# hiimmuc/SpeakerVerification

Hardware: AMD Instinct MI355X
Metric: embeddings/sec (2 s @16 kHz) (higher is better)
Workload: dtype bf16

## Files before the change

### speakerverification_amd/csrc/api.hip

```cpp
#include <algorithm>
#include <cstdlib>
#include <cstring>

#include "handle.h"

using namespace svhip;

namespace svhip {
RaggedCheckFn ecapa_ragged_check, rawnet2_ragged_check, rawnet3_ragged_check, conformer_ragged_check, titanet_ragged_check, resnetse_ragged_check;
RaggedEmbedFn ecapa_embed_ragged, rawnet2_embed_ragged, rawnet3_embed_ragged, conformer_embed_ragged, titanet_embed_ragged, resnetse_embed_ragged;
}

namespace {

thread_local std::string g_create_error;

enum DevOptParse { OPT_NO_ENV, OPT_SET, OPT_IS1, OPT_NUM };
struct DevOptRow { const char* name; int svhip_handle::DevOpts::*field; const char* env; DevOptParse parse; int dflt; };
#define SV_OPT(name, env, parse, dflt) {#name, &svhip_handle::DevOpts::name, env, parse, dflt}
const DevOptRow kDevOpts[] = {
    SV_OPT(layer_labels, "SVHIP_LAYER_LABELS", OPT_SET, 0),
    SV_OPT(x3_keep_f32, "SVHIP_X3_KEEP_F32", OPT_SET, 0),
    SV_OPT(r2_big, "SVHIP_R2_BIG", OPT_IS1, 0),
    SV_OPT(asp_v1, "SVHIP_ASP_V1", OPT_IS1, 0),
// ... 5 lines not shown
    SV_OPT(asnorm_norefit, nullptr, OPT_NO_ENV, 0),
    SV_OPT(rn_sinc_full, "SVHIP_RN_SINC_FULL", OPT_IS1, 0),
    SV_OPT(fbank32, "SVHIP_FBANK32", OPT_IS1, 0),
    SV_OPT(fbank_unfused, "SVHIP_FBANK_UNFUSED", OPT_IS1, 0),
    SV_OPT(pw3_cus, "SVHIP_PW3_CUS", OPT_NUM, -1),
    SV_OPT(pw3_tail_off, "SVHIP_PW3_TAIL_OFF", OPT_IS1, 0),
    SV_OPT(cv_off, "SVHIP_CV_OFF", OPT_IS1, 0),
    SV_OPT(n128_off, "SVHIP_N128_OFF", OPT_IS1, 0),
    SV_OPT(rn_pool_off, "SVHIP_RN_POOL_OFF", OPT_IS1, 0),
    SV_OPT(rn_step_off, "SVHIP_RN_STEP_OFF", OPT_IS1, 0),
    SV_OPT(rn_sinc_f32, "SVHIP_RN_SINC_F32", OPT_IS1, 0),
    SV_OPT(rn_tail_big, "SVHIP_RN_TAIL_BIG", OPT_IS1, 0),
    SV_OPT(r2_slices, "SVHIP_R2_SLICES", OPT_NUM, -1),
    SV_OPT(rn_conv_unfused, "SVHIP_RN_CONV_UNFUSED", OPT_IS1, 0),
    SV_OPT(rn_keep, "SVHIP_RN_KEEP", OPT_IS1, 0),
};
#undef SV_OPT

int none_check(const svhip_config& c, const char*& err) {
    if (c.compute == SVHIP_F16) { err = "SVHIP_F16 is RawNet2's 16-bit mode (ECAPA's is SVHIP_BF16)"; return SVHIP_ERR_UNSUPPORTED; }
    return SVHIP_OK;
}
int fbank_then_features(svhip_handle* h, const float* d_wav, int B);

const ModelOps kModels[] = {
    {SVHIP_MODEL_ECAPA,        ecapa_check,     ecapa_spec,     ecapa_finalize,     ecapa_alloc,     ecapa_embed_wave,    ecapa_forward,     ecapa_stage,     2,
     nullptr, ecapa_ragged_check, ecapa_embed_ragged},
    {SVHIP_MODEL_RAWNET2,      rawnet2_check,   rawnet2_spec,   rawnet2_finalize,   rawnet2_alloc,   rawnet2_forward,     nullptr,           rawnet2_stage,   4},
    {SVHIP_MODEL_RAWNET2_CONV, rawnet2_check,   rawnet2_spec,   rawnet2_finalize,   rawnet2_alloc,   rawnet2_forward,     nullptr,           rawnet2_stage,   4,
     nullptr, rawnet2_ragged_check, rawnet2_embed_ragged},
// ... 661 lines not shown
```

### speakerverification_amd/csrc/api_ecapa.hip

```cpp
#include <algorithm>

#include "handle.h"

namespace svhip {

namespace {

struct EcapaState : ModelState {
    ConvLayer blocks0, mfa, asp_tdnn, asp_conv;
    ConvLayer tdnn1[3], tdnn2[3], res2[3][7];
    LinearLayer se1[3], se2[3], asp_ctx, fc;
    float* se2T[3] = {};
    void *se1_bf[3] = {}, *se2T_bf[3] = {};
    float *aspbn_scale = nullptr, *aspbn_shift = nullptr;

    bool xin_ready = false;
    bool x0_is_s32 = false;
    bool cat_f32_stale = false;
    bool h2_is_s32 = false;
    bool h1_split = false;
    void* cat_s32 = nullptr;
    void* h2_s32 = nullptr;
    void* u_s32[2] = {};
    void* X0 = nullptr;
    void *H1 = nullptr, *H2 = nullptr, *H3 = nullptr;
    void* CAT = nullptr;
    void* MFA = nullptr;
    void* ATT = nullptr;
    float* LOGITS = nullptr;
    float *d_mean = nullptr, *d_s1 = nullptr, *d_s2 = nullptr, *d_gstats = nullptr, *d_ctx = nullptr;
    float *d_pool_raw = nullptr, *d_pool_bn = nullptr;

    RagTables rag;
    float* rag_stats = nullptr;
};
// ... 208 lines not shown
            GemmParams q = conv_params(h, L, us[(j - 1) & 1], C8, h2s + (size_t)j * C8 * 4, C, M, T);
            q.W = L.Ws32; q.Wrows = L.N; q.x3 = 2; q.act1 = ACT_RELU;
            if (j < 7) { q.R = static_cast<const float*>(H1) + (size_t)(j + 1) * C8; q.ldr = C; q.Y2 = us[j & 1]; q.lda2 = C8; }
            return q;
        };
        GemmParams p2 = conv_params(h, s.tdnn2[i], H2, C, H3, C, M, T);
        p2.act1 = ACT_GELU;
        p2.colsum = cs_base; p2.colsum_stride = h->colsum_region;
        const bool r2_small = h->x3 && h2s && us[0] && us[1] && s.res2[i][0].Ws32 && !h->opt.r2_big && r2_step_supported(step_params(1)) &&
                              conv_plan(h, s.tdnn2[i], p2, h2s, C).x3;
        const bool r2_plan = r2_small || (h->x3 && h2s && us[0] && us[1] && s.res2[i][0].Ws32 && gemm_pw3r2_supported(step_params(1)));
        GemmParams p1 = tdnn1_params(i, (s32_only && (i > 0 || x0_s32)) ? nullptr : xin, ldin);
        if (r2_plan) {
            p1.side_a = h2s; p1.side_lda = C; p1.side_b = us[0]; p1.side_ldb = C8; p1.side_c = C8;
        }
        GemmPlan g1;
        if ((rc = conv_gemm(h, s.tdnn1[i], p1, xin32, ldin32, &g1))) return rc;
        if (i == 2) { s.h2_is_s32 = r2_plan; s.h1_split = r2_plan && g1.side; }
        if (r2_plan) {
            if (!g1.side) {
                if ((rc = run(h, "split_s32", 0, [&]() { return launch_split_s32(static_cast<const float*>(H1), C, h2s, M, C8, st, C); }))) return rc;
                if ((rc = run(h, "split_s32", 0, [&]() { return launch_split_s32(static_cast<const float*>(H1) + C8, C, us[0], M, C8, st, C8); }))) return rc;
            }
            for (int j = 1; j < 8; ++j) {
                const GemmParams q = step_params(j);
                if (r2_small) {
                    if ((rc = run(h, "r2_step", (double)M * s.res2[i][j - 1].flops_per_row, [&]() { return launch_r2_step(q, st); }))) return rc;
                } else if ((rc = run(h, "gemm_pw3r2", (double)M * s.res2[i][j - 1].flops_per_row, [&]() { return launch_gemm_pw3r2(q, st); }))) return rc;
            }
            p2.A = nullptr;
        } else if (bf && res2net_chain_supported(C, T, s.res2[i][0].dil, s.res2[i][0].Kp)) {
            Res2Params rp;
            rp.H1 = H1; rp.H2 = H2; rp.ld = C; rp.T = T; rp.dil = s.res2[i][0].dil; rp.Kp = s.res2[i][0].Kp;
            rp.slices = h->opt.r2_slices >= 0 ? std::max(1, h->opt.r2_slices) : res2net_chain_slices(B, C, T, rp.dil, h->num_cu);
            double fl = 0;
            for (int j = 0; j < 7; ++j) {
                rp.W[j] = s.res2[i][j].W; rp.bias[j] = s.res2[i][j].bias;
                rp.scale[j] = s.res2[i][j].scale; rp.shift[j] = s.res2[i][j].shift;
                fl += (double)M * s.res2[i][j].flops_per_row;
            }
            if ((rc = run(h, rp.slices > 1 ? "res2net_slices" : "res2net_chain", fl, [&]() { return launch_res2net_chain(rp, B, C, st); }))) return rc;
        } else {
            if ((rc = run(h, "copy_cols", 0, [&]() { return launch_copy_cols(H1, C, H2, C, bf, M, C8, st); }))) return rc;
            for (int j = 1; j < 8; ++j) {
                GemmParams p = conv_params(h, s.res2[i][j - 1], off(H1, (size_t)j * C8, e), C, off(H2, (size_t)j * C8, e), C, M, T);
                p.act1 = ACT_RELU;
                p.A2 = j >= 2 ? off(H2, (size_t)(j - 1) * C8, e) : nullptr; p.lda2 = C;
                if ((rc = conv_gemm(h, s.res2[i][j - 1], p))) return rc;
// ... 59 lines not shown
        GemmParams p = conv_params(h, s.asp_conv, ATT, 128, LOGITS, C3, M, T);
        p.out_f32 = 1;
        if ((rc = conv_gemm(h, s.asp_conv, p))) return rc;
        if ((rc = run(h, "asp_pool", 0, [&]() {
                 return launch_asp_pool(LOGITS, MFA, bf, C3, B, T, C3, s.aspbn_scale, s.aspbn_shift, d_pool_raw, d_pool_bn, 1e-12f, 0.0f, st);
             }))) return rc;
    }
    if ((rc = run(h, "fc", 2.0 * B * s.fc.N * s.fc.K, [&]() {
             return launch_rowvec_linear(d_pool_bn, 2 * C3, s.fc.W, s.fc.bias, d_emb, c.embed_dim, B, c.embed_dim, 2 * C3, ACT_NONE, st, h->d_lin_part + (size_t)b0 * h->lin_part_per_utt);
         }))) return rc;
    return SVHIP_OK;
}

int ecapa_forward(svhip_handle* h, const float* d_feat, int B) {
    S(h).cat_f32_stale = false;
    const bool two = h->lanes == 2 && B >= 64 && !h->x3;
    return forward_lanes(h, ecapa_forward_part, d_feat, B, two ? 2 : 1, (B / 2 + 3) & ~3);
}

int ecapa_embed_wave(svhip_handle* h, const float* d_wav, int B) {
    auto& s = S(h);
    const int L = h->cfg.samples, T = h->T;
    const bool fused = h->bf16 && !h->in_w && h->d_logmel && !h->opt.fbank_unfused && !h->opt.fbank32 && fbank_fused_supported(h->fb, L);
    int rc;
    if (fused) {
        if ((rc = run(h, "fbank_fused", 0, [&]() {
                 return launch_fbank_fused(h->fb, d_wav, B, L, T, h->cfg.log_input, h->d_logmel, h->d_fpart, h->X_in, h->stream);
             }))) return rc;
    } else if ((rc = run(h, "fbank", 0, [&]() { return launch_fbank(h->fb, d_wav, B, L, T, h->d_feat, h->stream); }))) return rc;
    s.xin_ready = fused;
// ... 77 lines not shown
         }))) return rc;
    return run(h, "rag_fc", 2.0 * n * s.fc.N * s.fc.K, [&]() {
        return launch_rag_linear(s.d_pool_bn, 2 * C3, s.fc.W, s.fc.bias, h->d_emb, c.embed_dim, n, c.embed_dim, 2 * C3, ACT_NONE, st);
    });
}

int ecapa_embed_ragged(svhip_handle* h, const float* in, bool in_host, bool is_wave, const int64_t* in_off, const int32_t* lengths, int n) {
    auto& s = S(h);
    const size_t B = h->cfg.max_batch, utt_cap[RAG_LEVELS] = {B * (size_t)h->T};
    RagPack pk;
    int rc;
    if (!s.rag_stats && (rc = dev_alloc(h, &s.rag_stats, B * h->cfg.n_mels * 2))) return rc;
    if ((rc = rag_pack(h, s.rag, kEcapaRag, utt_cap, in, in_host, is_wave, in_off, lengths, n, pk)) || (rc = ecapa_forward_ragged(h, pk))) return rc;
    set_rag_rows(h, pk);
    s.x0_is_s32 = s.cat_f32_stale = s.h2_is_s32 = s.h1_split = false;
    return SVHIP_OK;
}

int ecapa_stage(svhip_handle* h, const std::string& n, bool fill, StageView& v) {
    auto& s = S(h);
    const int C = h->cfg.channels, C3 = 3 * C, B = h->lastB;
    const int64_t M = (int64_t)B * h->T;
    if (n == "blocks.0") {
        v.src = s.X0; v.cols = v.ld = C;
        if (s.x0_is_s32 && fill) {
            SV_HIP(h, launch_unsplit_s32(s.X0, C, static_cast<float*>(h->s32_buf), C, M, C, h->stream));
            v.src = h->s32_buf;
        }
    } else if (n == "blocks.1" || n == "blocks.2" || n == "blocks.3") {
        const int i = n.back() - '1';
        v.src = off(s.CAT, (size_t)i * C, h->esz); v.cols = C; v.ld = C3;
        if (s.cat_f32_stale && fill) {
            SV_HIP(h, launch_unsplit_s32(s.cat_s32, C3, static_cast<float*>(s.CAT), C3, M, C3, h->stream));
            s.cat_f32_stale = false;
        }
    }
    else if (n == "blocks.3.tdnn1") {
        if (s.h1_split)
            SV_FAIL(h, SVHIP_ERR_STATE, "stage blocks.3.tdnn1: the last forward wrote its first two chunks only in the split layout of the "
                                        "Res2Net step kernels, which the chain then overwrote");
        v.src = s.H1; v.cols = v.ld = C;
    } else if (n == "blocks.3.res2net") {
        v.src = s.H2; v.cols = v.ld = C;
        if (s.h2_is_s32 && fill) {
            SV_HIP(h, launch_unsplit_s32(s.h2_s32, C, static_cast<float*>(h->s32_buf), C, M, C, h->stream));
            v.src = h->s32_buf;
        }
    }
    else if (n == "blocks.3.tdnn2") { v.src = s.H3; v.cols = v.ld = C; }
    else if (n == "blocks.3.se_gate") { v.src = s.d_s2; v.rows = B; v.cols = v.ld = C; v.f32 = true; }
    else if (n == "asp_gstats") { v.src = s.d_gstats; v.rows = B; v.cols = v.ld = 2 * C3; v.f32 = true; }
    else if (n == "asp_att") { v.src = s.ATT; v.cols = v.ld = 128; }
    else if (n == "mfa") { v.src = s.MFA; v.cols = v.ld = C3; }
    else if (n == "asp") { v.src = s.d_pool_raw; v.rows = B; v.cols = v.ld = 2 * C3; v.f32 = true; }
    else if (n == "asp_bn") { v.src = s.d_pool_bn; v.rows = B; v.cols = v.ld = 2 * C3; v.f32 = true; }
    else return unknown_stage(h, n);
// ... 5 lines not shown
```

### speakerverification_amd/csrc/api_gemm.hip

```cpp
#include "handle.h"

namespace svhip {

static const void* zero_page_for(const svhip_handle* h, const void* A) {
    const char* a = static_cast<const char*>(A);
    for (const TailedBuf& b : h->tailed)
        if (a >= b.base && a < b.base + b.bytes) return b.base + b.bytes;
    return h->d_zero;
}

GemmParams conv_params(const svhip_handle* h, const ConvLayer& L, const void* A, int lda, void* Y, int ldy, int M, int T) {
    GemmParams p;
    p.A = A; p.lda = lda; p.Y = Y; p.ldy = ldy;
    p.W = L.W; p.Wrows = L.Np; p.bias = L.bias; p.scale = L.scale; p.shift = L.shift;
    p.M = M; p.N = L.N; p.K = L.K; p.Kp = L.Kp; p.T = T; p.taps = L.taps; p.dil = L.dil; p.cin = L.cin;
    p.num_cu = h->num_cu; p.pw3_cus = h->opt.pw3_cus; p.tail_split = h->opt.pw3_tail_off ? 0 : 1;
    p.zeros = h->d_zeros; p.ones = h->d_ones; p.f16 = h->f16 ? 1 : 0;
    p.cv_off = h->opt.cv_off; p.n128_off = h->opt.n128_off;
    return p;
}

GemmPlan conv_plan(const svhip_handle* h, const ConvLayer& L, GemmParams p, const void* A_s32, int lda_s32) {
    GemmPlan g;
    p.zero_page = zero_page_for(h, p.A);
    const int M = p.M;
    const bool bf = h->bf16;
    g.flops = (double)M * (L.flops_per_row + 2.0 * L.N * p.K3);
    if (h->x3 && L.Ws32 && h->s32_buf && !p.A2 && !p.bias_utt && !p.out_f32 && !p.R) {
        GemmParams q = p;
        q.A = A_s32 ? A_s32 : h->s32_buf; q.lda = A_s32 ? lda_s32 : L.K; q.W = L.Ws32; q.x3 = 2;
        if (!gemm_pw3x3_supported(q)) q.side_a = q.side_b = nullptr, q.side_c = 0;
        if (!gemm_pw3x3_supported(q) && q.colsum) q.colsum = nullptr;
        if (gemm_pw3x3_supported(q)) {
            g.q = q; g.x3 = true; g.side = q.side_c != 0; g.colsum_groups = q.colsum ? 2 : 0;
            snprintf(g.label, sizeof(g.label), "gemm_pw3x3");
            return g;
        }
    }
    if (h->x3) {
        p.x3 = 1;
        if (gemm_pw_supported(p, false) && L.Wsplit) p.W = L.Wsplit;
    }
    if (p.colsum) {
        if (gemm_pw2_supported(p, bf) && p.taps == 1) g.colsum_groups = gemm_colsum_groups(p, bf);
        else p.colsum = nullptr;
    }
    g.q = p;
    const GemmRoute route = g.route = gemm_route(p, bf);
    const char* klabel = route == ROUTE_PW3 ? "gemm_pw3" : route == ROUTE_PW3CV ? "gemm_pw3cv16" : route == ROUTE_N128 ? "gemm_n128" : route == ROUTE_PW2 ? (L.taps > 1 ? "gemm_pw2_conv" : "gemm_pw2")
                         : L.taps > 1 ? (p.A2 ? "gemm_conv_add" : "gemm_conv") : (route == ROUTE_GENERIC ? "gemm_generic" : "gemm_pw");
    if (!h->opt.layer_labels) snprintf(g.label, sizeof(g.label), "%s", klabel);
    else if (!p.K3) snprintf(g.label, sizeof(g.label), "%s M%d N%d K%d", klabel, M, L.N, L.K);
    else snprintf(g.label, sizeof(g.label), "%s M%d N%d K%d+%d", klabel, M, L.N, L.K, p.K3);
    return g;
}

int conv_gemm(svhip_handle* h, const ConvLayer& L, const GemmParams& p, const void* A_s32, int lda_s32, GemmPlan* plan) {
    const GemmPlan g = conv_plan(h, L, p, A_s32, lda_s32);
    if (plan) *plan = g;
    hipStream_t st = h->cur;
    if (g.x3) {
        int rc = A_s32 ? SVHIP_OK
                       : run(h, "split_s32", 0, [&]() { return launch_split_s32(reinterpret_cast<const float*>(p.A), p.lda, h->s32_buf, p.M, L.K, st); });
        return rc ? rc : run(h, g.label, g.flops, [&]() { return launch_gemm_pw3x3(g.q, st); });
    }
    if (!p.A)
// ... 7 lines not shown
```

### speakerverification_amd/csrc/gemm_pw3.hip

```cpp
#include <stdlib.h>

#include <type_traits>

#include "common.h"
#include "kernels.h"
#include "gemm_epi.h"

namespace svhip {

namespace {

typedef __attribute__((address_space(3))) void lds_void;
typedef __attribute__((address_space(1))) const void gbl_void;

constexpr int HT = 16384;
constexpr int RING = 8 * HT;
constexpr int CST = 3072;
constexpr int PW3_LDS = RING + 2 * CST;
constexpr int PGROUP_M = 8;

#ifdef SVHIP_GEMM_DEBUG
constexpr bool DBG3 = true;
#else
constexpr bool DBG3 = false;
#endif
#ifdef PW3_ABL
constexpr int ABL = PW3_ABL;
#else
constexpr int ABL = 0;
#endif

template <int EPI, int CS, bool X3, bool R2 = false, bool CV = false, typename H = bf16_t>
__global__ __launch_bounds__(512, 2) void gemm_pw3_kernel(GemmParams p) {
    static_assert(!R2 || (X3 && CS == 0), "the Res2Net step form exists for the X3 kernel only");
    static_assert(!CV || !R2, "the conv-gather form (CV) is the pointwise kernel with gathered X rows");
    typedef typename std::conditional<X3, x3_t, H>::type MH;
    constexpr bool GATHER = R2 || CV;
    extern __shared__ __attribute__((aligned(16))) char smem[];
    constexpr int NST = (X3 ? 32 : 16) + 8 * CS;
    constexpr int ESZ = X3 ? 4 : 2;

    const int ntm = (p.M + 255) / 256, ntn = (p.N + 255) / 256;
    const int ntiles = ntm * ntn;
    const int G = gridDim.x;
    int perm = blockIdx.x;
    {
        const int q = G >> 3, r = G & 7, xcd = perm & 7;
        perm = (xcd < r ? xcd * (q + 1) : r * (q + 1) + (xcd - r) * q) + (perm >> 3);
    }
    constexpr bool SPLIT_OK = !R2 && !(X3 && CV);
    const int qfull = (ntiles / G) * G;
    const int rtail = ntiles - qfull;
    const bool split = SPLIT_OK && p.tail_split && rtail > 0 && 2 * rtail <= G;
    const int nitems = split ? qfull + 2 * rtail : ntiles;
    auto item_tile = [&](int w, int& hsel) {
// ... 62 lines not shown
            uint32_t o = ty < 2 ? xo[ty][jj] : wo[ty - 2][jj];
            if (gather) {
                const int t = (int)((xt[jj] >> (ty * 16)) & 0xffffu);
                if (CV && !X3) {
                    const int tt = t + shift;
                    const int d = zero_pad ? shift : reflect_idx(tt, p.T) - t;
                    const uint32_t oo = (uint32_t)((int)o + d * p.lda * ESZ);
                    o = (zero_pad && (unsigned)tt >= (unsigned)p.T) ? zoff : oo;
                } else {
                    const int d = reflect_idx(t + shift, p.T) - t;
                    o = (uint32_t)((int)o + d * p.lda * ESZ);
                }
            }
            asm volatile("" : "+v"(o));
            const char* s = ub + o;
            if (!(ABL & 2)) __builtin_amdgcn_global_load_lds((gbl_void*)s, (lds_void*)(base + dsto[jj]), 16, 0, 0);
        }
    };
    auto issue_consts = [&](int n0, int par) {
        if (wave < 3) {
            const float* s = (wave == 0 ? p.bias : wave == 1 ? p.scale : p.shift) + min(n0 + lane_now() * 4, p.N - 4);
            __builtin_amdgcn_global_load_lds((gbl_void*)s, (lds_void*)(smem + RING + par * CST + wave * 1024), 16, 0, 0);
        }
    };
    auto issue_prologue = [&]() {
        issue(2, 0); issue(0, 0); issue(3, 0); issue(1, 0);
        issue(2, 1); issue(0, 1); issue(3, 1);
    };
    auto wait_left = [&](int left) {
        if (left >= 5) asm volatile("s_waitcnt vmcnt(10)" ::: "memory");
        else if (left == 4) asm volatile("s_waitcnt vmcnt(8)" ::: "memory");
// ... 296 lines not shown
                    const int m = m0 + wm * 128 + i * 16 + r16e;
                    const bool in = m < p.M && !(ABL & 8);
                    if (side_chunk < 2) {
                        uint32_t hd[2], ld[2];
#pragma unroll
                        for (int d = 0; d < 2; ++d) x3_split2(v[2 * d], v[2 * d + 1], hd[d], ld[d]);
                        const auto s0 = __builtin_amdgcn_permlane16_swap(hd[0], ld[0], false, false);
                        const auto s1 = __builtin_amdgcn_permlane16_swap(hd[1], ld[1], false, false);
                        if (in) *reinterpret_cast<u32x4*>(sbase + (int64_t)m * sld + boff) = u32x4{s0[0], s1[0], s0[1], s1[1]};
                    } else if (in) {
                        *reinterpret_cast<f32x4*>(yl + (int64_t)i * 16 * p.ldy) = v;
                    }
                }
            }
        } else {
            char* Yb = reinterpret_cast<char*>(p.Y);
#pragma unroll
            for (int jp = 0; jp < 2; ++jp) {
                if (half && jp == 1) break;
                f32x4 sc[2], sh[2];
#pragma unroll
                for (int jj = 0; jj < 2; ++jj) {
                    const int nl = wn * 64 + (2 * jp + jj) * 16 + 4 * q4e;
                    sc[jj] = *reinterpret_cast<const f32x4*>(cb + 1024 + nl * 4);
                    sh[jj] = *reinterpret_cast<const f32x4*>(cb + 2048 + nl * 4);
                }
                const int c0 = n0 + wn * 64 + jp * 32 + (q4e & 1) * 16 + (q4e >> 1) * 8;
                char* yl = Yb + ((int64_t)(m0 + wm * 128 + r16e) * p.ldy + c0) * 2;
#pragma unroll
                for (int i = 0; i < 8; ++i) {
                    float v0[4], v1[4];
                    if (ABL & 4) {
#pragma unroll
                        for (int e = 0; e < 4; ++e) { v0[e] = acc16[i][2 * jp][e]; v1[e] = acc16[i][2 * jp + 1][e]; }
                    } else {
                        act4<EPI>(v0, acc16[i][2 * jp], sc[0], sh[0]);
                        act4<EPI>(v1, acc16[i][2 * jp + 1], sc[1], sh[1]);
                    }
                    if (CS) {
                        acc16[i][2 * jp] = f32x4{v0[0], v0[1], v0[2], v0[3]};
                        acc16[i][2 * jp + 1] = f32x4{v1[0], v1[1], v1[2], v1[3]};
                    }
                    const auto s0 = __builtin_amdgcn_permlane16_swap(Half16<H>::pack2(v0[0], v0[1]), Half16<H>::pack2(v1[0], v1[1]), false, false);
                    const auto s1 = __builtin_amdgcn_permlane16_swap(Half16<H>::pack2(v0[2], v0[3]), Half16<H>::pack2(v1[2], v1[3]), false, false);
                    const int m = m0 + wm * 128 + i * 16 + r16e;
                    if (m < p.M && !(ABL & 8))
                        *reinterpret_cast<u32x4*>(yl + (int64_t)i * 16 * p.ldy * 2) = u32x4{s0[0], s1[0], s0[1], s1[1]};
                }
            }
        }
        if (CS) {
            const int lo = wm * 128;
            const int rb = (m0 / p.T + 1) * p.T - m0;
            const int rend = min(256, p.M - m0);
            const bool whole = (lo + 128 <= rend) && (lo + 128 <= rb || lo >= rb);
            float* csp = p.colsum + ((int64_t)(tm * 2 + wm) * 2) * p.N + n0 + wn * 64 + 4 * q4e;
            const f32x4 zero4 = {0.f, 0.f, 0.f, 0.f};
            const int jn = half ? 2 : 4;
            auto fresh_zero4 = [&]() { float z = 0.f; asm volatile("" : "+v"(z)); return f32x4{z, z, z, z}; };
            if (whole) {
                const int sg = lo >= rb ? 1 : 0;
#pragma unroll
// ... 143 lines not shown
    if (p.taps > 1 || p.R || p.A3 || p.f16) return false;
    if (!pw3_offsets_fit(p, 2)) return false;
    if (p.N % 256 != 0 || p.Kp < 256) return false;
    if (!p.bias || !p.scale || !p.shift) return false;
    if (p.act2 != ACT_NONE || !(p.act1 == ACT_NONE || p.act1 == ACT_RELU || p.act1 == ACT_GELU)) return false;
    if (p.num_cu <= 0 || p.num_cu > 1024) return false;
    const int ntiles = ((p.M + 255) / 256) * (p.N / 256);
    return ntiles > pw3_grid_cap(p) || (p.tail_split && 2 * ntiles <= pw3_grid_cap(p) && pw3_grid_cap(p) <= p.num_cu);
}

int pw3_grid_cap(const GemmParams& p) {
    if (p.pw3_cus == 0) return 1 << 30;
    return p.pw3_cus > 0 ? (p.pw3_cus < p.num_cu ? p.pw3_cus : p.num_cu) : p.num_cu;
}

hipError_t launch_gemm_pw3(const GemmParams& p, hipStream_t stream) {
    if (!gemm_pw3_supported(p, true) || p.M <= 0 || p.Wrows < p.N) return hipErrorInvalidValue;
    switch (p.act1) {
        case ACT_NONE: return launch_cs<EPI_NONE, false>(p, stream);
        case ACT_RELU: return launch_cs<EPI_RELU, false>(p, stream);
        case ACT_GELU: return launch_cs<EPI_GELU, false>(p, stream);
        default: return hipErrorInvalidValue;
    }
}

bool gemm_pw3x3_supported(const GemmParams& p) {
    if (p.x3 != 2 || p.out_f32 || p.bias_utt || p.A2 || p.A3 || p.R || p.taps > 1 || p.y_s32) return false;
    if (!pw3_offsets_fit(p, 4)) return false;
    if (p.act1 != ACT_GELU || p.act2 != ACT_NONE) return false;
    if (!p.bias || !p.scale || !p.shift) return false;
    if (p.N % 256 != 0 || p.K != p.Kp || p.K % 64 != 0 || p.K < 128 || p.lda < p.K || p.lda % 32 != 0 || p.ldy % 4 != 0) return false;
    if (p.colsum && (p.T < 256 || p.M % p.T != 0)) return false;
// ... 97 lines not shown
```

### speakerverification_amd/csrc/handle.h

```cpp
#pragma once
#include "../../include/svhip.h"

#include <hip/hip_runtime.h>

#include <cstdio>
#include <initializer_list>
#include <map>
#include <memory>
#include <string>
#include <vector>

#include "common.h"
#include "kernels.h"

namespace svhip {

struct HostTensor {
    std::vector<float> data;
    std::vector<int64_t> shape;
    int64_t numel() const { int64_t n = 1; for (auto s : shape) n *= s; return n; }
};

struct ConvLayer {
    int N = 0, K = 0, Kp = 0, Np = 0, taps = 1, dil = 1, cin = 0;
// ... 46 lines not shown
        int asnorm_norefit;
        int rn_sinc_full;
        int fbank32;
        int fbank_unfused;
        int pw3_cus;
        int pw3_tail_off;
        int cv_off;
        int n128_off;
        int rn_pool_off;
        int rn_step_off;
        int rn_sinc_f32;
        int rn_tail_big;
        int r2_slices;
        int rn_conv_unfused;
        int rn_keep;
    } opt;
    bool bf16 = false;
    bool f16 = false;
    int dt = svhip::DT_F32;
    bool x3 = false;
    bool finalized = false;
    std::string err;
    std::map<std::string, svhip::HostTensor> host_w;
    std::vector<void*> allocs;

    int T = 0;
    int esz = 4;

    svhip::FbankTables fb;
    int num_cu = 256;
// ... 177 lines not shown
             const int64_t* in_off, const int32_t* lengths, int n, RagPack& pk);
inline void set_rag_rows(svhip_handle* h, const RagPack& pk) {
    h->lastB = pk.n;
    h->rag_levels = pk.levels;
    for (int l = 0; l < pk.levels; ++l) h->rag_rows[l] = pk.lv[l].M;
}
using RagUttRule = int(int64_t bound, int i, int64_t T, std::string& err);
int rag_mel_check(const svhip_config& c, const int32_t* lengths, int n, bool is_wave, std::string& err, bool cfg_extra_ok, const char* cfg_names,
                  int min_frames, const char* why, RagUttRule* more = nullptr, int64_t bound = 0, int row_unit = 1);

struct GemmPlan {
    GemmParams q;
    bool x3 = false;
    GemmRoute route = ROUTE_GENERIC;
    bool side = false;
    int colsum_groups = 0;
    double flops = 0;
    char label[96] = "";
};
GemmParams conv_params(const svhip_handle* h, const ConvLayer& L, const void* A, int lda, void* Y, int ldy, int M, int T);
GemmPlan conv_plan(const svhip_handle* h, const ConvLayer& L, GemmParams p, const void* A_s32 = nullptr, int lda_s32 = 0);
int conv_gemm(svhip_handle* h, const ConvLayer& L, const GemmParams& p, const void* A_s32 = nullptr, int lda_s32 = 0, GemmPlan* plan = nullptr);

using ForwardPart = int (*)(svhip_handle* h, const float* in, int b0, int B);
int forward_lanes(svhip_handle* h, ForwardPart part, const float* in, int B, int lanes, int per);

CheckFn ecapa_check, rawnet2_check, rawnet3_check, titanet_check, conformer_check, resnetse_check;
SpecFn ecapa_spec, rawnet2_spec, rawnet3_spec, titanet_spec, conformer_spec, resnetse_spec;
HandleFn ecapa_finalize, rawnet2_finalize, rawnet3_finalize, titanet_finalize, conformer_finalize, resnetse_finalize;
HandleFn ecapa_alloc, rawnet2_alloc, rawnet3_alloc, titanet_alloc, conformer_alloc, resnetse_alloc;
// ... 10 lines not shown
```

### speakerverification_amd/csrc/kernels.h

```cpp
#pragma once
#include <hip/hip_runtime.h>
#include <stdint.h>

#include <atomic>

#include "common.h"

namespace svhip {

struct DeviceOnce {
    std::atomic<uint64_t> mask{0};
    bool done(int dev) const { return dev >= 0 && dev < 64 && ((mask.load(std::memory_order_acquire) >> dev) & 1u); }
    void mark(int dev) { if (dev >= 0 && dev < 64) mask.fetch_or(1ull << dev, std::memory_order_release); }
};
inline hipError_t set_max_dynamic_lds(DeviceOnce& once, const void* fn, int bytes) {
    int dev = -1;
    hipError_t e = hipGetDevice(&dev);
    if (e != hipSuccess) return e;
    if (once.done(dev)) return hipSuccess;
    e = hipFuncSetAttribute(fn, hipFuncAttributeMaxDynamicSharedMemorySize, bytes);
    if (e == hipSuccess) once.mark(dev);
    return e;
}

// ... 9 lines not shown
    float* colsum = nullptr;
    int colsum_sq = 0;
    int64_t colsum_stride = 0;
    const float* zeros = nullptr;
    const float* ones = nullptr;
    const void* zero_page = nullptr;
    void* Y2 = nullptr;
    const void* R = nullptr;
    int ldr = 0;
    const void* A3 = nullptr;
    int lda3 = 0, K3 = 0;
    int y_s32 = 0;
    void* side_a = nullptr;
    void* side_b = nullptr;
    int side_lda = 0, side_ldb = 0, side_c = 0;
    int num_cu = 256;
    int n128_off = 0;
    int cv_off = 0;
    int pw3_cus = -1;
    const float* in_scale = nullptr;
    int tail_split = 1;
    void* ts = nullptr;
    int M = 0, N = 0, K = 0, Kp = 0;
    int lda = 0, lda2 = 0, ldy = 0, ld_bu = 0;
    int T = 1;
    uint32_t t_magic = 0;
    int taps = 1, dil = 1, cin = 0, pad_mode = 0;
    int act1 = 0, act2 = 0;
    int out_f32 = 0;
    int f16 = 0;
// ... 12 lines not shown
constexpr int GEMM_BN = 128;
constexpr int GEMM_BK_BYTES = 128;

inline int gemm_bk(bool bf16) { return bf16 ? 64 : 32; }
inline int round_up(int x, int m) { return (x + m - 1) / m * m; }

hipError_t launch_gemm(const GemmParams& p, bool bf16, hipStream_t stream);
enum GemmRoute : int { ROUTE_PW2 = 0, ROUTE_PW = 1, ROUTE_PW_NARROW = 2, ROUTE_GENERIC = 3, ROUTE_PW3 = 4, ROUTE_PW3CV = 5, ROUTE_N128 = 6 };
GemmRoute gemm_route(const GemmParams& p, bool bf16);
bool gemm_pw_supported(const GemmParams& p, bool bf16);
hipError_t launch_gemm_pw(const GemmParams& p, bool bf16, hipStream_t stream, bool narrow = false);
bool gemm_pw2_supported(const GemmParams& p, bool bf16);
hipError_t launch_gemm_pw2(const GemmParams& p, hipStream_t stream);
bool gemm_pw3_supported(const GemmParams& p, bool bf16);
hipError_t launch_gemm_pw3(const GemmParams& p, hipStream_t stream);
int pw3_grid_cap(const GemmParams& p);
bool gemm_pw3x3_supported(const GemmParams& p);
hipError_t launch_gemm_pw3x3(const GemmParams& p, hipStream_t stream);
bool r2_step_supported(const GemmParams& p);
hipError_t launch_r2_step(const GemmParams& p, hipStream_t stream);
bool rn_step_supported(const GemmParams& p, int mode);
hipError_t launch_rn_step(const GemmParams& p, int mode, hipStream_t stream);
bool gemm_pw3cv_supported(const GemmParams& p);
hipError_t launch_gemm_pw3cv(const GemmParams& p, hipStream_t stream);
bool gemm_n128_supported(const GemmParams& p);
hipError_t launch_gemm_n128(const GemmParams& p, hipStream_t stream);
bool gemm_pw3cv16_supported(const GemmParams& p);
hipError_t launch_gemm_pw3cv16(const GemmParams& p, hipStream_t stream);
bool gemm_pw3r2_supported(const GemmParams& p);
hipError_t launch_gemm_pw3r2(const GemmParams& p, hipStream_t stream);
// ... 16 lines not shown
hipError_t launch_rag_linear(const float* in, int ld_in, const float* W, const float* bias, float* out, int ld_out, int n, int N, int K,
                             int act, hipStream_t stream);

struct Res2Params {
    const void* H1 = nullptr;
    void* H2 = nullptr;
    int ld = 0, T = 0, dil = 1, Kp = 0;
    const void* W[7] = {};
    const float* bias[7] = {};
    const float* scale[7] = {};
    const float* shift[7] = {};
    int debug = 0;
    unsigned long long* ts = nullptr;
    int slices = 1;
    int Tc = 0;
};
bool res2net_chain_supported(int C, int T, int dil, int Kp);
int res2net_chain_slices(int B, int C, int T, int dil, int num_cu);
hipError_t launch_res2net_chain(const Res2Params& p, int B, int C, hipStream_t stream);

struct FbankTables {
    const float* basis = nullptr;
    const void* basis_hi = nullptr;
    const void* basis_lo = nullptr;
    const void* basis_l3 = nullptr;
    const void* sym_hi = nullptr;
    const void* sym_lo = nullptr;
    int split6 = 0;
    int n_k16 = 13;
    int split_bf16 = 0;
// ... 301 lines not shown
```

### speakerverification_amd/csrc/res2net.hip

```cpp
#include "common.h"
#include "kernels.h"

namespace svhip {

namespace {

#ifdef SVHIP_GEMM_DEBUG
constexpr bool R2DBG = true;
#else
constexpr bool R2DBG = false;
#endif
constexpr int R2_TMAX = 416;

template <int CW, int MIT> struct R2Cfg {
    static constexpr int ROWB = CW * 2;
    static constexpr int NCH = ROWB / 16;
    static constexpr int NT = CW / 32;
    static constexpr int MW = 8 / NT;
    static constexpr int MI = MIT;
    static constexpr int TMAX = MW * MI * 32 < R2_TMAX ? MW * MI * 32 : R2_TMAX;
    static constexpr int U_BYTES = TMAX * ROWB;
    static constexpr int W_BYTES = CW * ROWB;
    static constexpr int LDS = U_BYTES + W_BYTES;
    static constexpr int WCH = CW * NCH / 512;
    static __device__ __forceinline__ int swz(int row) { return CW == 128 ? (row & 15) : ((row >> 1) & 7); }
// ... 40 lines not shown
        for (int e = 0; e < WCH; ++e) {
            const int c = tid_w + 512 * e;
            const int n = c / NCH, ch = c % NCH;
            *reinterpret_cast<u32x4*>(Wt + n * ROWB + ((ch ^ CF::swz(n)) << 4)) = wregs[e];
        }
    };

    wload(0, 0);
    {
        constexpr int RSTEP = 512 / NCH, RB0 = 4;
        const int row0 = tid / NCH, ch0 = tid % NCH;
        const uint32_t goff0 = ((uint32_t)row0 * (uint32_t)p.ld + (uint32_t)ch0 * 8u) * 2u;
        const uint32_t gstep = (uint32_t)RSTEP * (uint32_t)p.ld * 2u;
        const char* h1b = reinterpret_cast<const char*>(H1);
        char* h2b = reinterpret_cast<char*>(H2);
        for (int it0 = 0; it0 * RSTEP < T; it0 += RB0) {
            u32x4 cc0[RB0], cc1[RB0];
#pragma unroll
            for (int k = 0; k < RB0; ++k)
                if (row0 + (it0 + k) * RSTEP < T) {
                    cc0[k] = __builtin_nontemporal_load(reinterpret_cast<const u32x4*>(h1b + goff0 + (uint32_t)(it0 + k) * gstep));
                    cc1[k] = __builtin_nontemporal_load(reinterpret_cast<const u32x4*>(h1b + CW * 2 + goff0 + (uint32_t)(it0 + k) * gstep));
                }
#pragma unroll
            for (int k = 0; k < RB0; ++k) {
                const int row = row0 + (it0 + k) * RSTEP;
                if (row < T) {
                    if (row >= s0 && row < s1) *reinterpret_cast<u32x4*>(h2b + goff0 + (uint32_t)(it0 + k) * gstep) = cc0[k];
                    *reinterpret_cast<u32x4*>(U + row * ROWB + ((ch0 ^ CF::swz(row)) << 4)) = cc1[k];
                }
            }
        }
    }
    wstore();
    __syncthreads();
    const bool stamp = R2DBG && (p.debug & 64) && p.ts && tid == 0;
    unsigned long long tprev = 0;
    if (R2DBG && (p.debug & 64) && p.ts) tprev = __builtin_readcyclecounter();
    if (stamp) p.ts[(size_t)blockIdx.x * 32 + 3] = tprev;
#define R2_STAMP(stage, k) if (R2DBG && (p.debug & 64) && p.ts) { const unsigned long long t_ = __builtin_readcyclecounter(); if (stamp) p.ts[(size_t)blockIdx.x * 32 + (stage) * 4 + (k)] = t_ - tprev; tprev = t_; }

    for (int s = 1; s < 8; ++s) {
        const int layer = s - 1;
// ... 101 lines not shown
            asm volatile("" : "+v"(tid_r));
            const int row0 = tid_r / NCH, ch0 = tid_r % NCH;
            const uint32_t goff0 = ((uint32_t)row0 * (uint32_t)p.ld + (uint32_t)ch0 * 8u) * 2u;
            const uint32_t gstep = (uint32_t)RSTEP * (uint32_t)p.ld * 2u;
            char* h2s = reinterpret_cast<char*>(H2) + s * CW * 2;
#pragma unroll
            for (int g = 0; g < NPRE / RB; ++g) {
                const int it0 = g * RB;
                if (it0 * RSTEP < T) {
#pragma unroll
                    for (int k = 0; k < RB; ++k) {
                        const int row = row0 + (it0 + k) * RSTEP;
                        if (row < T) {
                            char* up = U + row * ROWB + ((ch0 ^ CF::swz(row)) << 4);
                            const bf16x8 y = *reinterpret_cast<const bf16x8*>(up);
                            if (!noglob && row >= s0 && row < s1) *reinterpret_cast<bf16x8*>(h2s + goff0 + (uint32_t)(it0 + k) * gstep) = y;
                            if (s < 7 && !noglob) {
                                const bf16x8 cv = __builtin_bit_cast(bf16x8, cpre[it0 + k]);
                                bf16x8 u;
#pragma unroll
                                for (int e = 0; e < 8; ++e) u[e] = static_cast<bf16_t>(static_cast<float>(y[e]) + static_cast<float>(cv[e]));
                                *reinterpret_cast<bf16x8*>(up) = u;
                            }
                        }
                    }
                }
            }
        }
        __syncthreads();
        R2_STAMP(s, 2)
    }
// ... 49 lines not shown
```

Before: 58570.

## Write Res2Net chunk 0 directly from tdnn1 GEMM; add nontemporal cache policies

The tdnn1 pw3 GEMM now writes its first C/8 output columns (Res2Net chunk 0, which passes through unchanged) straight into H2. The Res2Net chain kernel no longer has to reload and copy that chunk from H1. The stage-dump path restores H1's chunk 0 afterward when layer outputs are inspected. It also adds compile-time cache-policy selection: nontemporal loads for one operand in the plain pw3 GEMM (default POL=2) and nontemporal stores for the per-step H2 slice writes in the chain kernel. The intent is to cut redundant global traffic and cache pollution, at the cost of extra bookkeeping and the hazard that H1 chunk 0 is never written when the split path runs.

Result: no change. 59320 (median of 6 runs) (+1.3%).

```diff
diff --git a/speakerverification_amd/csrc/api.hip b/speakerverification_amd/csrc/api.hip
--- a/speakerverification_amd/csrc/api.hip
+++ b/speakerverification_amd/csrc/api.hip
@@ -43,6 +43,7 @@
     SV_OPT(r2_slices, "SVHIP_R2_SLICES", OPT_NUM, -1),
     SV_OPT(rn_conv_unfused, "SVHIP_RN_CONV_UNFUSED", OPT_IS1, 0),
     SV_OPT(rn_keep, "SVHIP_RN_KEEP", OPT_IS1, 0),
+    SV_OPT(c0_split_off, "SVHIP_C0_SPLIT_OFF", OPT_IS1, 0),
 };
 #undef SV_OPT
 
diff --git a/speakerverification_amd/csrc/api_ecapa.hip b/speakerverification_amd/csrc/api_ecapa.hip
--- a/speakerverification_amd/csrc/api_ecapa.hip
+++ b/speakerverification_amd/csrc/api_ecapa.hip
@@ -19,6 +19,8 @@
     bool cat_f32_stale = false;
     bool h2_is_s32 = false;
     bool h1_split = false;
+    size_t c0_row0[2] = {};
+    int c0_rows[2] = {};
     void* cat_s32 = nullptr;
     void* h2_s32 = nullptr;
     void* u_s32[2] = {};
@@ -257,9 +259,12 @@
         if (r2_plan) {
             p1.side_a = h2s; p1.side_lda = C; p1.side_b = us[0]; p1.side_ldb = C8; p1.side_c = C8;
         }
+        const bool chain = !r2_plan && bf && res2net_chain_supported(C, T, s.res2[i][0].dil, s.res2[i][0].Kp);
+        if (chain && !h->opt.c0_split_off) { p1.Y_lo = H2; p1.ld_lo = C; p1.n_lo = C8; }
         GemmPlan g1;
         if ((rc = conv_gemm(h, s.tdnn1[i], p1, xin32, ldin32, &g1))) return rc;
         if (i == 2) { s.h2_is_s32 = r2_plan; s.h1_split = r2_plan && g1.side; }
+        if (i == 2) { s.c0_row0[b0 ? 1 : 0] = r0; s.c0_rows[b0 ? 1 : 0] = g1.lo ? M : 0; }
         if (r2_plan) {
             if (!g1.side) {
                 if ((rc = run(h, "split_s32", 0, [&]() { return launch_split_s32(static_cast<const float*>(H1), C, h2s, M, C8, st, C); }))) return rc;
@@ -272,9 +277,10 @@
                 } else if ((rc = run(h, "gemm_pw3r2", (double)M * s.res2[i][j - 1].flops_per_row, [&]() { return launch_gemm_pw3r2(q, st); }))) return rc;
             }
             p2.A = nullptr;
-        } else if (bf && res2net_chain_supported(C, T, s.res2[i][0].dil, s.res2[i][0].Kp)) {
+        } else if (chain) {
             Res2Params rp;
             rp.H1 = H1; rp.H2 = H2; rp.ld = C; rp.T = T; rp.dil = s.res2[i][0].dil; rp.Kp = s.res2[i][0].Kp;
+            rp.c0_done = g1.lo ? 1 : 0;
             rp.slices = h->opt.r2_slices >= 0 ? std::max(1, h->opt.r2_slices) : res2net_chain_slices(B, C, T, rp.dil, h->num_cu);
             double fl = 0;
             for (int j = 0; j < 7; ++j) {
@@ -364,6 +370,7 @@
 
 int ecapa_forward(svhip_handle* h, const float* d_feat, int B) {
     S(h).cat_f32_stale = false;
+    S(h).c0_rows[0] = S(h).c0_rows[1] = 0;
     const bool two = h->lanes == 2 && B >= 64 && !h->x3;
     return forward_lanes(h, ecapa_forward_part, d_feat, B, two ? 2 : 1, (B / 2 + 3) & ~3);
 }
@@ -471,6 +478,7 @@
     if ((rc = rag_pack(h, s.rag, kEcapaRag, utt_cap, in, in_host, is_wave, in_off, lengths, n, pk)) || (rc = ecapa_forward_ragged(h, pk))) return rc;
     set_rag_rows(h, pk);
     s.x0_is_s32 = s.cat_f32_stale = s.h2_is_s32 = s.h1_split = false;
+    s.c0_rows[0] = s.c0_rows[1] = 0;
     return SVHIP_OK;
 }
 
@@ -497,6 +505,11 @@
             SV_FAIL(h, SVHIP_ERR_STATE, "stage blocks.3.tdnn1: the last forward wrote its first two chunks only in the split layout of the "
                                         "Res2Net step kernels, which the chain then overwrote");
         v.src = s.H1; v.cols = v.ld = C;
+        for (int l = 0; l < 2 && fill; ++l)
+            if (s.c0_rows[l]) {
+                SV_HIP(h, launch_copy_cols(off(s.H2, s.c0_row0[l] * C, h->esz), C, off(s.H1, s.c0_row0[l] * C, h->esz), C, h->bf16, s.c0_rows[l], C / 8, h->stream));
+                s.c0_rows[l] = 0;
+            }
     } else if (n == "blocks.3.res2net") {
         v.src = s.H2; v.cols = v.ld = C;
         if (s.h2_is_s32 && fill) {
diff --git a/speakerverification_amd/csrc/api_gemm.hip b/speakerverification_amd/csrc/api_gemm.hip
--- a/speakerverification_amd/csrc/api_gemm.hip
+++ b/speakerverification_amd/csrc/api_gemm.hip
@@ -29,6 +29,7 @@
     if (h->x3 && L.Ws32 && h->s32_buf && !p.A2 && !p.bias_utt && !p.out_f32 && !p.R) {
         GemmParams q = p;
         q.A = A_s32 ? A_s32 : h->s32_buf; q.lda = A_s32 ? lda_s32 : L.K; q.W = L.Ws32; q.x3 = 2;
+        q.Y_lo = nullptr; q.ld_lo = q.n_lo = 0;
         if (!gemm_pw3x3_supported(q)) q.side_a = q.side_b = nullptr, q.side_c = 0;
         if (!gemm_pw3x3_supported(q) && q.colsum) q.colsum = nullptr;
         if (gemm_pw3x3_supported(q)) {
@@ -47,9 +48,12 @@
     }
     g.q = p;
     const GemmRoute route = g.route = gemm_route(p, bf);
+    g.lo = route == ROUTE_PW3 && p.n_lo > 0 && gemm_pw3_lo_ok(p);
+    if (!g.lo) { g.q.Y_lo = nullptr; g.q.ld_lo = g.q.n_lo = 0; }
     const char* klabel = route == ROUTE_PW3 ? "gemm_pw3" : route == ROUTE_PW3CV ? "gemm_pw3cv16" : route == ROUTE_N128 ? "gemm_n128" : route == ROUTE_PW2 ? (L.taps > 1 ? "gemm_pw2_conv" : "gemm_pw2")
                          : L.taps > 1 ? (p.A2 ? "gemm_conv_add" : "gemm_conv") : (route == ROUTE_GENERIC ? "gemm_generic" : "gemm_pw");
     if (!h->opt.layer_labels) snprintf(g.label, sizeof(g.label), "%s", klabel);
+    else if (g.lo) snprintf(g.label, sizeof(g.label), "%s M%d N%d K%d lo%d", klabel, M, L.N, L.K, p.n_lo);
     else if (!p.K3) snprintf(g.label, sizeof(g.label), "%s M%d N%d K%d", klabel, M, L.N, L.K);
     else snprintf(g.label, sizeof(g.label), "%s M%d N%d K%d+%d", klabel, M, L.N, L.K, p.K3);
     return g;
diff --git a/speakerverification_amd/csrc/gemm_pw3.hip b/speakerverification_amd/csrc/gemm_pw3.hip
--- a/speakerverification_amd/csrc/gemm_pw3.hip
+++ b/speakerverification_amd/csrc/gemm_pw3.hip
@@ -29,6 +29,11 @@
 #else
 constexpr int ABL = 0;
 #endif
+#ifdef PW3_POL
+constexpr int POL = PW3_POL;
+#else
+constexpr int POL = 2;
+#endif
 
 template <int EPI, int CS, bool X3, bool R2 = false, bool CV = false, typename H = bf16_t>
 __global__ __launch_bounds__(512, 2) void gemm_pw3_kernel(GemmParams p) {
@@ -39,6 +44,9 @@
     extern __shared__ __attribute__((aligned(16))) char smem[];
     constexpr int NST = (X3 ? 32 : 16) + 8 * CS;
     constexpr int ESZ = X3 ? 4 : 2;
+    constexpr bool PLAIN16 = !X3 && !R2 && !CV;
+    constexpr int X_AUX = (PLAIN16 && ((POL >> CS) & 1)) ? CPOL_NT : 0, W_AUX = (PLAIN16 && (POL & 64)) ? CPOL_NT : 0;
+    constexpr bool Y_NT = PLAIN16 && ((POL >> (3 + CS)) & 1);
 
     const int ntm = (p.M + 255) / 256, ntn = (p.N + 255) / 256;
     const int ntiles = ntm * ntn;
@@ -131,7 +139,10 @@
             }
             asm volatile("" : "+v"(o));
             const char* s = ub + o;
-            if (!(ABL & 2)) __builtin_amdgcn_global_load_lds((gbl_void*)s, (lds_void*)(base + dsto[jj]), 16, 0, 0);
+            if (!(ABL & 2)) {
+                if (X_AUX != W_AUX && ty < 2) __builtin_amdgcn_global_load_lds((gbl_void*)s, (lds_void*)(base + dsto[jj]), 16, 0, X_AUX);
+                else __builtin_amdgcn_global_load_lds((gbl_void*)s, (lds_void*)(base + dsto[jj]), 16, 0, W_AUX);
+            }
         }
     };
     auto issue_consts = [&](int n0, int par) {
@@ -458,7 +469,8 @@
                 }
             }
         } else {
-            char* Yb = reinterpret_cast<char*>(p.Y);
+            const bool to_lo = !CV && n0 + wn * 64 < p.n_lo;
+            char* Yb = reinterpret_cast<char*>(to_lo ? p.Y_lo : p.Y);
 #pragma unroll
             for (int jp = 0; jp < 2; ++jp) {
                 if (half && jp == 1) break;
@@ -488,8 +500,11 @@
                     const auto s0 = __builtin_amdgcn_permlane16_swap(Half16<H>::pack2(v0[0], v0[1]), Half16<H>::pack2(v1[0], v1[1]), false, false);
                     const auto s1 = __builtin_amdgcn_permlane16_swap(Half16<H>::pack2(v0[2], v0[3]), Half16<H>::pack2(v1[2], v1[3]), false, false);
                     const int m = m0 + wm * 128 + i * 16 + r16e;
-                    if (m < p.M && !(ABL & 8))
-                        *reinterpret_cast<u32x4*>(yl + (int64_t)i * 16 * p.ldy * 2) = u32x4{s0[0], s1[0], s0[1], s1[1]};
+                    if (m < p.M && !(ABL & 8)) {
+                        u32x4* dst = reinterpret_cast<u32x4*>(yl + (int64_t)i * 16 * p.ldy * 2);
+                        if (Y_NT) __builtin_nontemporal_store(u32x4{s0[0], s1[0], s0[1], s1[1]}, dst);
+                        else *dst = u32x4{s0[0], s1[0], s0[1], s1[1]};
+                    }
                 }
             }
         }
@@ -663,8 +678,13 @@
     return p.pw3_cus > 0 ? (p.pw3_cus < p.num_cu ? p.pw3_cus : p.num_cu) : p.num_cu;
 }
 
+bool gemm_pw3_lo_ok(const GemmParams& p) {
+    return (p.n_lo == 64 || p.n_lo == 128) && p.n_lo <= p.N && p.Y_lo && p.ld_lo == p.ldy && p.ld_lo >= p.n_lo && p.ld_lo % 8 == 0 &&
+           (reinterpret_cast<uintptr_t>(p.Y_lo) & 15) == 0;
+}
+
 hipError_t launch_gemm_pw3(const GemmParams& p, hipStream_t stream) {
-    if (!gemm_pw3_supported(p, true) || p.M <= 0 || p.Wrows < p.N) return hipErrorInvalidValue;
+    if (!gemm_pw3_supported(p, true) || p.M <= 0 || p.Wrows < p.N || (p.n_lo && !gemm_pw3_lo_ok(p))) return hipErrorInvalidValue;
     switch (p.act1) {
         case ACT_NONE: return launch_cs<EPI_NONE, false>(p, stream);
         case ACT_RELU: return launch_cs<EPI_RELU, false>(p, stream);
diff --git a/speakerverification_amd/csrc/handle.h b/speakerverification_amd/csrc/handle.h
--- a/speakerverification_amd/csrc/handle.h
+++ b/speakerverification_amd/csrc/handle.h
@@ -84,6 +84,7 @@
         int r2_slices;
         int rn_conv_unfused;
         int rn_keep;
+        int c0_split_off;
     } opt;
     bool bf16 = false;
     bool f16 = false;
@@ -291,6 +292,7 @@
     bool x3 = false;
     GemmRoute route = ROUTE_GENERIC;
     bool side = false;
+    bool lo = false;
     int colsum_groups = 0;
     double flops = 0;
     char label[96] = "";
diff --git a/speakerverification_amd/csrc/kernels.h b/speakerverification_amd/csrc/kernels.h
--- a/speakerverification_amd/csrc/kernels.h
+++ b/speakerverification_amd/csrc/kernels.h
@@ -47,6 +47,8 @@
     void* side_a = nullptr;
     void* side_b = nullptr;
     int side_lda = 0, side_ldb = 0, side_c = 0;
+    void* Y_lo = nullptr;
+    int ld_lo = 0, n_lo = 0;
     int num_cu = 256;
     int n128_off = 0;
     int cv_off = 0;
@@ -89,6 +91,7 @@
 hipError_t launch_gemm_pw2(const GemmParams& p, hipStream_t stream);
 bool gemm_pw3_supported(const GemmParams& p, bool bf16);
 hipError_t launch_gemm_pw3(const GemmParams& p, hipStream_t stream);
+bool gemm_pw3_lo_ok(const GemmParams& p);
 int pw3_grid_cap(const GemmParams& p);
 bool gemm_pw3x3_supported(const GemmParams& p);
 hipError_t launch_gemm_pw3x3(const GemmParams& p, hipStream_t stream);
@@ -135,6 +138,7 @@
     unsigned long long* ts = nullptr;
     int slices = 1;
     int Tc = 0;
+    int c0_done = 0;
 };
 bool res2net_chain_supported(int C, int T, int dil, int Kp);
 int res2net_chain_slices(int B, int C, int T, int dil, int num_cu);
diff --git a/speakerverification_amd/csrc/res2net.hip b/speakerverification_amd/csrc/res2net.hip
--- a/speakerverification_amd/csrc/res2net.hip
+++ b/speakerverification_amd/csrc/res2net.hip
@@ -9,6 +9,11 @@
 constexpr bool R2DBG = true;
 #else
 constexpr bool R2DBG = false;
+#endif
+#ifdef R2_YS_NT
+constexpr bool YS_NT = R2_YS_NT != 0;
+#else
+constexpr bool YS_NT = true;
 #endif
 constexpr int R2_TMAX = 416;
 
@@ -79,19 +84,20 @@
         const uint32_t gstep = (uint32_t)RSTEP * (uint32_t)p.ld * 2u;
         const char* h1b = reinterpret_cast<const char*>(H1);
         char* h2b = reinterpret_cast<char*>(H2);
+        const bool copy_c0 = !p.c0_done;
         for (int it0 = 0; it0 * RSTEP < T; it0 += RB0) {
             u32x4 cc0[RB0], cc1[RB0];
 #pragma unroll
             for (int k = 0; k < RB0; ++k)
                 if (row0 + (it0 + k) * RSTEP < T) {
-                    cc0[k] = __builtin_nontemporal_load(reinterpret_cast<const u32x4*>(h1b + goff0 + (uint32_t)(it0 + k) * gstep));
+                    if (copy_c0) cc0[k] = __builtin_nontemporal_load(reinterpret_cast<const u32x4*>(h1b + goff0 + (uint32_t)(it0 + k) * gstep));
                     cc1[k] = __builtin_nontemporal_load(reinterpret_cast<const u32x4*>(h1b + CW * 2 + goff0 + (uint32_t)(it0 + k) * gstep));
                 }
 #pragma unroll
             for (int k = 0; k < RB0; ++k) {
                 const int row = row0 + (it0 + k) * RSTEP;
                 if (row < T) {
-                    if (row >= s0 && row < s1) *reinterpret_cast<u32x4*>(h2b + goff0 + (uint32_t)(it0 + k) * gstep) = cc0[k];
+                    if (copy_c0 && row >= s0 && row < s1) *reinterpret_cast<u32x4*>(h2b + goff0 + (uint32_t)(it0 + k) * gstep) = cc0[k];
                     *reinterpret_cast<u32x4*>(U + row * ROWB + ((ch0 ^ CF::swz(row)) << 4)) = cc1[k];
                 }
             }
@@ -223,7 +229,11 @@
                         if (row < T) {
                             char* up = U + row * ROWB + ((ch0 ^ CF::swz(row)) << 4);
                             const bf16x8 y = *reinterpret_cast<const bf16x8*>(up);
-                            if (!noglob && row >= s0 && row < s1) *reinterpret_cast<bf16x8*>(h2s + goff0 + (uint32_t)(it0 + k) * gstep) = y;
+                            if (!noglob && row >= s0 && row < s1) {
+                                bf16x8* dst = reinterpret_cast<bf16x8*>(h2s + goff0 + (uint32_t)(it0 + k) * gstep);
+                                if (YS_NT) __builtin_nontemporal_store(y, dst);
+                                else *dst = y;
+                            }
                             if (s < 7 && !noglob) {
                                 const bf16x8 cv = __builtin_bit_cast(bf16x8, cpre[it0 + k]);
                                 bf16x8 u;
```
